# tayloreisman16/LTE-GNU-Radio-Code

Hardware: AMD Instinct MI355X
Metric: IQ Msamples/s through RX FFT+equalize, 2048-pt/144-CP; %HBM roofline; 1/2/4/8 GPU (higher is better)
Workload: dtype f32; 1 GPU; 2048-pt FFT / 144-CP / Kd=1200 / 16-QAM, 4369 frames x 240 symbols (1,048,560 symbols), AWGN loopback; frames_per_gpu=4369, symbols_per_gpu=1048560, outputs=equalised symbols + packed bits, parallelism=frame-shard x1, sync_search=screened

## Files before the change

lte-gnu-radio-code_amd/csrc/rx_demod.hpp:

```cpp
#pragma once
#include <algorithm>
#include <atomic>
#include <cstdlib>
#include <type_traits>

#include "ofdm_launch.hpp"

#ifndef OFDM_NS_T128
#define OFDM_NS_T128 2
#endif
#ifndef OFDM_MINW_T128
#define OFDM_MINW_T128 3
#endif
#ifndef OFDM_FLAGS_T128
#define OFDM_FLAGS_T128 0u
#endif
#ifndef OFDM_FLAGS_T256
#define OFDM_FLAGS_T256 0u
#endif
#ifndef OFDM_LANE_TW
#define OFDM_LANE_TW 1
#endif
#ifndef OFDM_SCATTER_HOIST
#define OFDM_SCATTER_HOIST 1
#endif
#ifndef OFDM_SCATTER_SKIP
#define OFDM_SCATTER_SKIP 1
#endif

namespace ofdm {

__device__ __forceinline__ unsigned qpsk_axis_bit(float x) {
    constexpr float t = 1.41421354f;
    return unsigned(x < 0.f) ^ unsigned(fabsf(x) > t);
}

__device__ __noinline__ unsigned qpsk_bits_on_axis(float zx, float zy) {
    constexpr double A = 0x1.6a09e667f3bcdp-1, B = 0x1.6a09e667f3bccp-1, Cc = 0x1.6a09e667f3bcep-1;
    const double cx[4] = {A, A, -B, -Cc};
    const double cy[4] = {B, -B, A, -B};
    constexpr double K = 0x1.6a09e667f3bccp+0;
    const double x = double(zx), y = double(zy);
    int kbest = 0;
    double dbest = 0.0;
#pragma unroll
    for (int k = 0; k < 4; ++k) {
        const double ax = fabs(x - cx[k]), ay = fabs(y - cy[k]);
        const double mx = fmax(ax, ay), mn = fmin(ay, ax);
        const double r = mn / mx;
        const double d = sqrt(fma(r, r, 1.0)) * mx;
        if (k == 0 || d < dbest) {
            dbest = d;
            kbest = k;
        }
    }
    const double ex = fabs(x - cx[kbest]), ey = fabs(y - cy[kbest]);
    const bool q1 = x >= 0.0 && y >= 0.0;
    const bool q2 = !q1 && x <= 0.0 && y >= 0.0;
    const bool q3 = !q1 && !q2 && x <= 0.0 && y <= 0.0;
    const bool q4 = !q1 && !q2 && !q3 && x >= 0.0 && y <= 0.0;
    const bool re_pos = q1 || q4, im_pos = q1 || q2;
    const double fr = K - ex, fi = K - ey;
    const unsigned b0 = re_pos ? (fr < ex) : (ex < fr);
    const unsigned b1 = im_pos ? (fi < ey) : (ey < fi);
    return (b0 << 1) | b1;
}

template <int MOD>
__device__ __forceinline__ unsigned hard_bits(cf z) {
    if constexpr (MOD == 2) {
        if (z.x == 0.f || z.y == 0.f) return qpsk_bits_on_axis(z.x, z.y);
        return (qpsk_axis_bit(z.x) << 1) | qpsk_axis_bit(z.y);
    } else if constexpr (MOD == 1) {
        return z.x > 0.f;
    } else if constexpr (MOD == 4) {
        constexpr float t = 0.63245553203367588f;
        return (unsigned(z.x < 0.f) << 3) | (unsigned(z.y < 0.f) << 2) | (unsigned(fabsf(z.x) > t) << 1) |
               unsigned(fabsf(z.y) > t);
    } else {
        constexpr float a = 0.61721339984836765f;
        constexpr float c = 0.30860669992418382f;
        return (unsigned(z.x < 0.f) << 5) | (unsigned(z.y < 0.f) << 4) | (unsigned(fabsf(z.x) > a) << 3) |
               (unsigned(fabsf(z.y) > a) << 2) | (unsigned(fabsf(fabsf(z.x) - a) > c) << 1) |
               unsigned(fabsf(fabsf(z.y) - a) > c);
    }
}
__device__ __forceinline__ unsigned hard_bits_rt(cf z, int mod) {
    return mod == 2 ? hard_bits<2>(z) : mod == 1 ? hard_bits<1>(z) : mod == 4 ? hard_bits<4>(z) : hard_bits<6>(z);
}

template <int MOD, bool ASMB = true>
__device__ __forceinline__ unsigned pack4(const cf (&z)[4]) {
    unsigned w = 0;
    if constexpr (!ASMB) {
        w = (((((hard_bits<MOD>(z[0]) << MOD) | hard_bits<MOD>(z[1])) << MOD) | hard_bits<MOD>(z[2])) << MOD) | hard_bits<MOD>(z[3]);
    } else if constexpr (MOD == 4) {
        constexpr float t = 0.63245553203367588f;
        unsigned long long m0, m1, m2, m3;
#define OFDM_Q16(RE, IM)                                   \
    "v_cmp_gt_f32_e64 %1, 0, " RE "\n\t"                   \
    "v_cmp_gt_f32_e64 %2, 0, " IM "\n\t"                   \
    "v_cmp_gt_f32_e64 %3, |" RE "|, %13\n\t"               \
    "v_cmp_gt_f32_e64 %4, |" IM "|, %13\n\t"               \
    "v_addc_co_u32_e64 %0, %1, %0, %0, %1\n\t"             \
    "v_addc_co_u32_e64 %0, %2, %0, %0, %2\n\t"             \
    "v_addc_co_u32_e64 %0, %3, %0, %0, %3\n\t"             \
    "v_addc_co_u32_e64 %0, %4, %0, %0, %4\n\t"
        asm(OFDM_Q16("%5", "%6") OFDM_Q16("%7", "%8") OFDM_Q16("%9", "%10") OFDM_Q16("%11", "%12")
            : "+v"(w), "=&s"(m0), "=&s"(m1), "=&s"(m2), "=&s"(m3)
            : "v"(z[0].x), "v"(z[0].y), "v"(z[1].x), "v"(z[1].y), "v"(z[2].x), "v"(z[2].y), "v"(z[3].x), "v"(z[3].y), "s"(t));
#undef OFDM_Q16
    } else if constexpr (MOD == 6) {
        constexpr float a = 0.61721339984836765f;
        constexpr float c = 0.30860669992418382f;
        unsigned long long m0, m1, m2, m3, m4, m5;
        float tr, ti;
#define OFDM_Q64(RE, IM)                                   \
    "v_sub_f32_e64 %7, |" RE "|, %17\n\t"                  \
    "v_sub_f32_e64 %8, |" IM "|, %17\n\t"                  \
    "v_cmp_gt_f32_e64 %1, 0, " RE "\n\t"                   \
    "v_cmp_gt_f32_e64 %2, 0, " IM "\n\t"                   \
    "v_cmp_gt_f32_e64 %3, |" RE "|, %17\n\t"               \
    "v_cmp_gt_f32_e64 %4, |" IM "|, %17\n\t"               \
    "v_cmp_gt_f32_e64 %5, |%7|, %18\n\t"                   \
    "v_cmp_gt_f32_e64 %6, |%8|, %18\n\t"                   \
    "v_addc_co_u32_e64 %0, %1, %0, %0, %1\n\t"             \
    "v_addc_co_u32_e64 %0, %2, %0, %0, %2\n\t"             \
    "v_addc_co_u32_e64 %0, %3, %0, %0, %3\n\t"             \
    "v_addc_co_u32_e64 %0, %4, %0, %0, %4\n\t"             \
    "v_addc_co_u32_e64 %0, %5, %0, %0, %5\n\t"             \
    "v_addc_co_u32_e64 %0, %6, %0, %0, %6\n\t"
        asm(OFDM_Q64("%9", "%10") OFDM_Q64("%11", "%12") OFDM_Q64("%13", "%14") OFDM_Q64("%15", "%16")
            : "+v"(w), "=&s"(m0), "=&s"(m1), "=&s"(m2), "=&s"(m3), "=&s"(m4), "=&s"(m5), "=&v"(tr), "=&v"(ti)
            : "v"(z[0].x), "v"(z[0].y), "v"(z[1].x), "v"(z[1].y), "v"(z[2].x), "v"(z[2].y), "v"(z[3].x), "v"(z[3].y), "s"(a), "s"(c));
#undef OFDM_Q64
    } else if constexpr (MOD == 2) {
        constexpr float t = 1.41421354f;
        if (!(fabsf(z[0].x * z[0].y * z[1].x * z[1].y) > 0.f) || !(fabsf(z[2].x * z[2].y * z[3].x * z[3].y) > 0.f)) {
            bool tie = false;
#pragma unroll
            for (int e = 0; e < 4; ++e) tie |= (z[e].x == 0.f) | (z[e].y == 0.f);
            if (tie)
                return (((((hard_bits<2>(z[0]) << 2) | hard_bits<2>(z[1])) << 2) | hard_bits<2>(z[2])) << 2) | hard_bits<2>(z[3]);
        }
        unsigned long long m0, m1, m2, m3, m4, m5, m6, m7;
#define OFDM_QPSK2(RE0, IM0, RE1, IM1)                     \
    "v_cmp_gt_f32_e64 %1, 0, " RE0 "\n\t"                  \
    "v_cmp_gt_f32_e64 %2, |" RE0 "|, %17\n\t"              \
    "v_cmp_gt_f32_e64 %3, 0, " IM0 "\n\t"                  \
    "v_cmp_gt_f32_e64 %4, |" IM0 "|, %17\n\t"              \
    "v_cmp_gt_f32_e64 %5, 0, " RE1 "\n\t"                  \
    "v_cmp_gt_f32_e64 %6, |" RE1 "|, %17\n\t"              \
    "v_cmp_gt_f32_e64 %7, 0, " IM1 "\n\t"                  \
    "v_cmp_gt_f32_e64 %8, |" IM1 "|, %17\n\t"              \
    "s_xor_b64 %1, %1, %2\n\t"                             \
    "s_xor_b64 %3, %3, %4\n\t"                             \
    "s_xor_b64 %5, %5, %6\n\t"                             \
    "s_xor_b64 %7, %7, %8\n\t"                             \
    "s_nop 1\n\t"                                          \
    "v_addc_co_u32_e64 %0, %1, %0, %0, %1\n\t"             \
    "v_addc_co_u32_e64 %0, %3, %0, %0, %3\n\t"             \
    "v_addc_co_u32_e64 %0, %5, %0, %0, %5\n\t"             \
    "v_addc_co_u32_e64 %0, %7, %0, %0, %7\n\t"
        asm(OFDM_QPSK2("%9", "%10", "%11", "%12") OFDM_QPSK2("%13", "%14", "%15", "%16")
            : "+v"(w), "=&s"(m0), "=&s"(m1), "=&s"(m2), "=&s"(m3), "=&s"(m4), "=&s"(m5), "=&s"(m6), "=&s"(m7)
            : "v"(z[0].x), "v"(z[0].y), "v"(z[1].x), "v"(z[1].y), "v"(z[2].x), "v"(z[2].y), "v"(z[3].x), "v"(z[3].y), "s"(t)
            : "scc");
#undef OFDM_QPSK2
    } else {
        w = (((((hard_bits<MOD>(z[0]) << MOD) | hard_bits<MOD>(z[1])) << MOD) | hard_bits<MOD>(z[2])) << MOD) | hard_bits<MOD>(z[3]);
    }
    return w;
}

template <int MOD, bool ASMB = true>
__device__ __forceinline__ unsigned pack2(const cf (&z)[2]) {
    unsigned w = 0;
    if constexpr (!ASMB || MOD == 1) {
        w = (hard_bits<MOD>(z[0]) << MOD) | hard_bits<MOD>(z[1]);
    } else if constexpr (MOD == 4) {
        constexpr float t = 0.63245553203367588f;
        unsigned long long m0, m1, m2, m3;
#define OFDM_Q16(RE, IM)                                   \
    "v_cmp_gt_f32_e64 %1, 0, " RE "\n\t"                   \
    "v_cmp_gt_f32_e64 %2, 0, " IM "\n\t"                   \
    "v_cmp_gt_f32_e64 %3, |" RE "|, %9\n\t"                \
    "v_cmp_gt_f32_e64 %4, |" IM "|, %9\n\t"                \
    "v_addc_co_u32_e64 %0, %1, %0, %0, %1\n\t"             \
    "v_addc_co_u32_e64 %0, %2, %0, %0, %2\n\t"             \
    "v_addc_co_u32_e64 %0, %3, %0, %0, %3\n\t"             \
    "v_addc_co_u32_e64 %0, %4, %0, %0, %4\n\t"
        asm(OFDM_Q16("%5", "%6") OFDM_Q16("%7", "%8")
            : "+v"(w), "=&s"(m0), "=&s"(m1), "=&s"(m2), "=&s"(m3)
            : "v"(z[0].x), "v"(z[0].y), "v"(z[1].x), "v"(z[1].y), "s"(t));
#undef OFDM_Q16
    } else if constexpr (MOD == 6) {
        constexpr float a = 0.61721339984836765f;
        constexpr float c = 0.30860669992418382f;
        unsigned long long m0, m1, m2, m3, m4, m5;
        float tr, ti;
#define OFDM_Q64(RE, IM)                                   \
    "v_sub_f32_e64 %7, |" RE "|, %13\n\t"                  \
    "v_sub_f32_e64 %8, |" IM "|, %13\n\t"                  \
    "v_cmp_gt_f32_e64 %1, 0, " RE "\n\t"                   \
    "v_cmp_gt_f32_e64 %2, 0, " IM "\n\t"                   \
    "v_cmp_gt_f32_e64 %3, |" RE "|, %13\n\t"               \
    "v_cmp_gt_f32_e64 %4, |" IM "|, %13\n\t"               \
    "v_cmp_gt_f32_e64 %5, |%7|, %14\n\t"                   \
    "v_cmp_gt_f32_e64 %6, |%8|, %14\n\t"                   \
    "v_addc_co_u32_e64 %0, %1, %0, %0, %1\n\t"             \
    "v_addc_co_u32_e64 %0, %2, %0, %0, %2\n\t"             \
    "v_addc_co_u32_e64 %0, %3, %0, %0, %3\n\t"             \
    "v_addc_co_u32_e64 %0, %4, %0, %0, %4\n\t"             \
    "v_addc_co_u32_e64 %0, %5, %0, %0, %5\n\t"             \
    "v_addc_co_u32_e64 %0, %6, %0, %0, %6\n\t"
        asm(OFDM_Q64("%9", "%10") OFDM_Q64("%11", "%12")
            : "+v"(w), "=&s"(m0), "=&s"(m1), "=&s"(m2), "=&s"(m3), "=&s"(m4), "=&s"(m5), "=&v"(tr), "=&v"(ti)
            : "v"(z[0].x), "v"(z[0].y), "v"(z[1].x), "v"(z[1].y), "s"(a), "s"(c));
#undef OFDM_Q64
    } else {
        constexpr float t = 1.41421354f;
        if (!(fabsf(z[0].x * z[0].y * z[1].x * z[1].y) > 0.f)) {
            const bool tie = (z[0].x == 0.f) | (z[0].y == 0.f) | (z[1].x == 0.f) | (z[1].y == 0.f);
            if (tie) return (hard_bits<2>(z[0]) << 2) | hard_bits<2>(z[1]);
        }
        unsigned long long m0, m1, m2, m3, m4, m5, m6, m7;
        asm("v_cmp_gt_f32_e64 %1, 0, %9\n\t"
            "v_cmp_gt_f32_e64 %2, |%9|, %13\n\t"
            "v_cmp_gt_f32_e64 %3, 0, %10\n\t"
            "v_cmp_gt_f32_e64 %4, |%10|, %13\n\t"
            "v_cmp_gt_f32_e64 %5, 0, %11\n\t"
            "v_cmp_gt_f32_e64 %6, |%11|, %13\n\t"
            "v_cmp_gt_f32_e64 %7, 0, %12\n\t"
            "v_cmp_gt_f32_e64 %8, |%12|, %13\n\t"
            "s_xor_b64 %1, %1, %2\n\t"
            "s_xor_b64 %3, %3, %4\n\t"
            "s_xor_b64 %5, %5, %6\n\t"
            "s_xor_b64 %7, %7, %8\n\t"
            "s_nop 1\n\t"
            "v_addc_co_u32_e64 %0, %1, %0, %0, %1\n\t"
            "v_addc_co_u32_e64 %0, %3, %0, %0, %3\n\t"
            "v_addc_co_u32_e64 %0, %5, %0, %0, %5\n\t"
            "v_addc_co_u32_e64 %0, %7, %0, %0, %7\n\t"
            : "+v"(w), "=&s"(m0), "=&s"(m1), "=&s"(m2), "=&s"(m3), "=&s"(m4), "=&s"(m5), "=&s"(m6), "=&s"(m7)
            : "v"(z[0].x), "v"(z[0].y), "v"(z[1].x), "v"(z[1].y), "s"(t)
            : "scc");
    }
    return w;
}

template <int MOD>
__device__ __forceinline__ void store_bits_pair_unpacked(uint8_t* row, unsigned sym0, const cf (&z)[2]) {
    uint8_t* o = row + sym0 * unsigned(MOD);
#pragma unroll
    for (int e = 0; e < 2; ++e) {
        const unsigned hb = hard_bits<MOD>(z[e]);
#pragma unroll
        for (int b = 0; b < MOD; ++b) o[e * MOD + b] = uint8_t((hb >> (MOD - 1 - b)) & 1u);
    }
}

template <int MOD>
__device__ __forceinline__ void store_packed4(uint8_t* row, unsigned sym0, unsigned w) {
    uint8_t* o = row + (sym0 >> 2) * unsigned(MOD / 2);
    if constexpr (MOD == 2) {
        o[0] = uint8_t(w);
    } else if constexpr (MOD == 4) {
        *reinterpret_cast<uint16_t*>(o) = uint16_t(((w & 0xffu) << 8) | (w >> 8));
    } else {
        o[0] = uint8_t(w >> 16);
        o[1] = uint8_t(w >> 8);
        o[2] = uint8_t(w);
    }
}

template <int MOD, int BMODE, bool ASMB = true>
__device__ __forceinline__ void store_bits(uint8_t* bits, int64_t sym0, const cf (&z)[4], int cnt) {
    if constexpr (BMODE == 1) {
        store_packed4<MOD>(bits + (sym0 >> 2) * (MOD / 2), 0u, pack4<MOD, ASMB>(z));
    } else if constexpr (BMODE == 2) {
        uint8_t* o = bits + sym0 * MOD;
#pragma unroll
        for (int e = 0; e < 4; ++e) {
            if (e < cnt) {
                const unsigned hb = hard_bits<MOD>(z[e]);
#pragma unroll
                for (int b = 0; b < MOD; ++b) o[e * MOD + b] = uint8_t((hb >> (MOD - 1 - b)) & 1u);
            }
        }
    }
}

template <int N>
struct DemodGeom {
    static constexpr int T = Plan<N>::T;
    static constexpr int NS = (T >= 256) ? 1 : (T >= 128) ? OFDM_NS_T128 : (T >= 64 ? 2 : 64 / T);
    static constexpr int WG = T * NS;
    static constexpr int W1_OFF = WgLds<N>::STRIDE * NS;
    static constexpr int Q_OFF = W1_OFF + WgLds<N>::W1_ELEMS;
    static constexpr int G_OFF = Q_OFF + 2;
    static size_t lds_bytes(int Kd, bool glds) { return (size_t(G_OFF) + (glds ? ((Kd + 3) & ~3) : 0)) * sizeof(cf); }
    static constexpr int KD_LTE = (N >= 1024) ? N * 75 / 128 : 0;
};

enum DemodFlags : unsigned {
    DF_ROT = 1u << 0,
    DF_HG = 1u << 1,
    DF_UNITS = 1u << 15,
    DF_GAINS_GLOBAL = 1u << 2,
    DF_TEMPORAL_LD = 1u << 3,
    DF_TEMPORAL_ST = 1u << 11,
    DF_GENERIC_BITS = 1u << 4,
    DF_STAMP = 1u << 5,
    DF_NO_PIPE = 1u << 6,
    DF_L2_INPUT = 1u << 7,
    DF_LANE_TWIDDLES = 1u << 8,
    DF_PSUM_READBACK = 1u << 9,
    DF_GAINS_VGPR = 1u << 14,
    DF_FOUR_PER_LANE = 1u << 10,
};

template <int N, int MOD, int BMODE, int MINW, unsigned FLAGS = 0, int KD = 0>
__global__ void __launch_bounds__(DemodGeom<N>::WG, MINW) rx_demod_kernel(RxDev rx, DemodArgs a) {
    static_assert(KD >= 0 && KD <= N && KD % 4 == 0, "compile-time bin-list length");
    constexpr bool ROT = (FLAGS & DF_ROT) != 0, HG = (FLAGS & DF_HG) != 0, UNITS = (FLAGS & DF_UNITS) != 0,
                   GREG = (FLAGS & DF_GAINS_VGPR) != 0 && Plan<N>::T >= 64 && (FLAGS & DF_FOUR_PER_LANE) == 0 && !(MOD == 1 && BMODE == 1),
                   GLDS = (FLAGS & DF_GAINS_GLOBAL) == 0 && !GREG,
                   NTL = (FLAGS & DF_TEMPORAL_LD) == 0 && Plan<N>::T >= 64, NT = (FLAGS & DF_TEMPORAL_ST) == 0 && Plan<N>::T >= 64, ASMB = (FLAGS & DF_GENERIC_BITS) == 0, STAMP = (FLAGS & DF_STAMP) != 0,
                   PIPE = (FLAGS & DF_NO_PIPE) == 0, L2IN = (FLAGS & DF_L2_INPUT) != 0,
                   CT = (FLAGS & DF_LANE_TWIDDLES) == 0 && !OFDM_LANE_TW && Plan<N>::R0 == 16, PSE = (FLAGS & DF_PSUM_READBACK) == 0,
                   DENSE = Plan<N>::T >= 64 && (FLAGS & DF_FOUR_PER_LANE) == 0 && !(MOD == 1 && BMODE == 1);
    using PL = Plan<N>;
    using DG = DemodGeom<N>;
    constexpr int T = PL::T, P = PL::P, Q = P / 4, NS = DG::NS;
    extern __shared__ __attribute__((aligned(16))) char smem_raw[];
    const int tid = threadIdx.x;
    const int slot = (T >= 64) ? __builtin_amdgcn_readfirstlane(tid / T) : tid / T;
    const int t = tid % T;
    constexpr bool WL = T <= 64;
    cf* smem = reinterpret_cast<cf*>(smem_raw);
    cf* lds = smem + slot * WgLds<N>::STRIDE;
    float* red = reinterpret_cast<float*>(lds + WgLds<N>::ELEMS);
    cf* w1w = smem + DG::W1_OFF;
    if constexpr (PL::THREE) {
        for (int e = tid; e < WgLds<N>::W1_ELEMS; e += DG::WG) w1w[e] = w1_entry<N>(rx.tw, e);
    }
    const cf* w1tab = w1w;

    std::conditional_t<CT, CompactTwiddles<N>, LaneTwiddles<N>> tw;
    load_twiddles(tw, rx.tw, t);

    unsigned acc[8] = {0, 0, 0, 0, 0, 0, 0, 0};
    unsigned long long tprev = 0;
    auto stamp = [&](int i) {
        if constexpr (STAMP) {
            unsigned long long tn;
            asm volatile("s_memtime %0\n\ts_waitcnt lgkmcnt(0)" : "=s"(tn)::"memory");
            acc[i] += unsigned(tn - tprev);
            tprev = tn;
        }
    };
    if constexpr (STAMP) asm volatile("s_memtime %0\n\ts_waitcnt lgkmcnt(0)" : "=s"(tprev)::"memory");
    const int64_t n_chunks = int64_t(a.n_frames) * a.chunks_per_frame;
    int* const qslot = reinterpret_cast<int*>(smem + DG::Q_OFF);
    int64_t chunk = blockIdx.x;
    if (a.work) {
        if (tid == 0) *qslot = int(atomicAdd(a.work, 1u));
        __syncthreads();
        chunk = *qslot;
    }
    for (; chunk < n_chunks;) {
    const int frame = int(chunk / a.chunks_per_frame);
    const int cidx = int(chunk % a.chunks_per_frame);
    const int trips = (a.n_dsym + NS - 1) / NS;
    const int ds0 = int(int64_t(cidx) * trips / a.chunks_per_frame) * NS;
    const int ds1 = min(int(int64_t(cidx + 1) * trips / a.chunks_per_frame) * NS, a.n_dsym);
    constexpr bool active = true;

    const int Kd = KD > 0 ? KD : rx.Kd, L = rx.L, S = rx.S, D = rx.D;
    const int tsr0 = a.tsr[frame * 4 + 0];
    const bool frame_on = (HG || UNITS) ? (a.tsr[frame * 4 + 3] != 0) : true;
    const int src_frame = UNITS ? frame / a.units_per_frame : frame;
    const cf* frame_iq = a.iq + int64_t(L2IN ? (blockIdx.x & 7) : src_frame) * a.frame_stride;
    const cf* rotp = (UNITS && ROT) ? a.rot + int64_t(max(a.rot_idx[src_frame], 0)) * N : a.rot;

    const cf* gain = a.gain + int64_t(frame) * Kd;
    cf* glds = smem + DG::G_OFF;
    const cf* gsrc = GLDS ? glds : gain;
    if constexpr (GLDS) {
        for (int i = 2 * tid; i < Kd; i += 2 * DG::WG) *reinterpret_cast<float4*>(glds + i) = *reinterpret_cast<const float4*>(gain + i);
    }
    float4 greg[GREG ? Q : 1][2];
    if constexpr (GREG) {
#pragma unroll
        for (int q = 0; q < Q; ++q)
#pragma unroll
            for (int hx = 0; hx < 2; ++hx) {
                const int idx = 4 * T * q + 256 * (t >> 6) + 128 * hx + 2 * (t & 63);
                greg[q][hx] = idx < Kd ? *reinterpret_cast<const float4*>(gain + idx) : float4{0.f, 0.f, 0.f, 0.f};
            }
    }

    const float sqrt_kd = sqrtf(float(Kd));
    const int n_iter = (ds1 - ds0 + NS - 1) / NS;
    struct Sym {
        bool valid, compute;
        int64_t start, orow;
    };
    auto sym_of = [&](int it) {
        Sym sy;
        const int itr = it;
        const int ds = ds0 + itr * NS + slot;
        sy.valid = active && it < n_iter && ds < ds1;
        const int p = ds / D, n_ = ds - p * D;
        const int64_t pat_ptr = int64_t(tsr0) + int64_t(S) * L * (int64_t(p) * (S + D) + 1);
        sy.compute = sy.valid && (HG ? frame_on : (pat_ptr + N - 1 <= a.frame_len)) && (!UNITS || frame_on);
        sy.start = pat_ptr + int64_t(L) * n_;
        sy.orow = int64_t(frame) * a.rows_per_frame + (p * a.row_stride_pat + n_);
        return sy;
    };
    cf v[P];
    auto load_sym = [&](const Sym& sy) {
        if (sy.compute && sy.start >= 0 && sy.start + N <= a.frame_len) {
            const cf* src = frame_iq + sy.start + t;
#pragma unroll
            for (int n0 = 0; n0 < P; ++n0) v[n0] = NTL ? __builtin_nontemporal_load(src + T * n0) : src[T * n0];
            if constexpr (ROT) {
#pragma unroll
                for (int n0 = 0; n0 < P; ++n0) v[n0] = cmul(v[n0], rotp[t + T * n0]);
            }
        } else {
            const int64_t before = -sy.start, left = a.frame_len - sy.start;
            const int lo = int(before < 0 ? 0 : (before < N ? before : N)), hi = int(left < 0 ? 0 : (left < N ? left : N));
            const bool any = sy.compute && hi > lo;
            int tq = t;
            asm volatile("" : "+v"(tq));
#pragma unroll
            for (int n0 = 0; n0 < P; ++n0) {
                const int e = tq + T * n0;
                const cf x = any ? frame_iq[sy.start + min(max(e, lo), hi - 1)] : cf{0.f, 0.f};
                v[n0] = (any && e >= lo && e < hi) ? x : cf{0.f, 0.f};
                if constexpr (ROT) v[n0] = cmul(v[n0], rotp[tq + T * n0]);
            }
        }
    };

    Sym cur = sym_of(0);
    if constexpr (PIPE) load_sym(cur);
    if constexpr (WL) wg_barrier();
    for (int it = 0; it < n_iter; ++it) {
        if constexpr (!PIPE) {
            cur = sym_of(it);
            load_sym(cur);
        }
        const bool sym_valid = cur.valid, compute = cur.compute;
        const int64_t orow = cur.orow;
        stamp(0);
        if constexpr (STAMP) asm volatile("s_waitcnt vmcnt(0)" ::: "memory");
        stamp(1);
        if constexpr (STAMP) {
            fft_pass0_store<N>(v, lds, tw, t);
            wg_barrier();
            stamp(2);
            if constexpr (PL::THREE) {
                fft_pass1_load<N>(v, lds, t);
                wg_barrier();
                fft_pass1_store<N>(v, lds, w1tab, t);
                wg_barrier();
            }
            stamp(3);
            fft_last_load<N>(v, lds, t);
            fft_last_dft<N>(v);
        } else {
            wg_fft<N, decltype(tw), WL>(v, lds, tw, w1tab, t);
        }
        slot_sync<WL>();

        int Kd_ = Kd;
#if !OFDM_SCATTER_HOIST
        asm volatile("" : "+s"(Kd_));
#endif
        const int hk = Kd_ >> 1;
        const int off_neg = hk - N, off_pos = hk - 1;
        float pse = 0.f;
#pragma unroll
        for (int j = 0; j < PL::C; ++j) {
#pragma unroll
            for (int kl = 0; kl < PL::RL; ++kl) {
#if OFDM_SCATTER_SKIP
                if constexpr (T >= 64) {
                    const int base = T * j + PL::NC * kl;
                    if (base > hk && base + T - 1 < N - hk) continue;
                }
#endif
                const int k = (t + T * j) + PL::NC * kl;
#if OFDM_SCATTER_SKIP
                if constexpr (T >= 64) {
                    const int base = T * j + PL::NC * kl;
                    const bool all_pos = base >= 1 && base + T - 1 <= hk, all_neg = base >= N - hk && hk < N / 2;
                    if (all_pos || all_neg) {
                        lds[k + (all_neg ? off_neg : off_pos)] = v[out_slot<N>(j, kl)];
                        if constexpr (PSE) pse += cnorm2(v[out_slot<N>(j, kl)]);
                        continue;
                    }
                }
#endif
                int i = k + ((k >= N - hk) ? off_neg : off_pos);
                if (j == 0 && kl == 0) i = (k == 0) ? N : i;
                lds[i] = v[out_slot<N>(j, kl)];
                if constexpr (PSE) pse += (unsigned(i) < unsigned(Kd_)) ? cnorm2(v[out_slot<N>(j, kl)]) : 0.f;
            }
        }
        if (Kd_ == N) {
#pragma unroll
            for (int j = 0; j < PL::C; ++j) {
#pragma unroll
                for (int kl = 0; kl < PL::RL; ++kl)
                    if ((t + T * j) + PL::NC * kl == N / 2) {
                        lds[N - 1] = v[out_slot<N>(j, kl)];
                        if constexpr (PSE) pse += cnorm2(v[out_slot<N>(j, kl)]);
                    }
            }
        }
        if constexpr (PSE) {
            pse = lanes_sum<T>(pse);
            if constexpr (T > 64) {
                if ((t & 63) == 0) red[t >> 6] = pse;
            }
        }
        slot_sync<WL>();

        stamp(4);
        if constexpr (PIPE) {
            cur = sym_of(it + 1);
            load_sym(cur);
        }
        float psum = 0.f;
        if constexpr (PSE) {
            if constexpr (T > 64) {
#pragma unroll
                for (int w = 0; w < T / 64; ++w) psum += red[w];
            } else {
                psum = pse;
            }
        } else {
#pragma unroll
            for (int q = 0; q < Q; ++q) {
                const int idx = 4 * (t + T * q);
                const float4 a01 = *reinterpret_cast<const float4*>(lds + idx);
                const float4 a23 = *reinterpret_cast<const float4*>(lds + idx + 2);
                const float p4[4] = {a01.x * a01.x + a01.y * a01.y, a01.z * a01.z + a01.w * a01.w,
                                     a23.x * a23.x + a23.y * a23.y, a23.z * a23.z + a23.w * a23.w};
                if (4 * T * (q + 1) <= Kd_) {
#pragma unroll
                    for (int e = 0; e < 4; ++e) psum += p4[e];
                } else {
#pragma unroll
                    for (int e = 0; e < 4; ++e) psum += (idx + e < Kd_) ? p4[e] : 0.f;
                }
            }
            psum = lanes_sum<T>(psum);
            if constexpr (T > 64) {
                if ((t & 63) == 0) red[t >> 6] = psum;
                wg_barrier();
                psum = 0.f;
#pragma unroll
                for (int w = 0; w < T / 64; ++w) psum += red[w];
            }
        }
        const float scale = sqrt_kd * __builtin_amdgcn_rsqf(psum);
        stamp(5);

        if (!compute) {
            if (sym_valid && a.zero_skipped) {
                const cf zz[4] = {cf{0.f, 0.f}, cf{0.f, 0.f}, cf{0.f, 0.f}, cf{0.f, 0.f}};
                int tq = t;
                asm volatile("" : "+v"(tq));
#pragma unroll
                for (int q = 0; q < Q; ++q) {
                    const int idx = 4 * (tq + T * q);
                    if (idx < Kd_) {
                        const bool four = idx + 2 < Kd_;
                        if (a.eq) {
                            float4* o = reinterpret_cast<float4*>(a.eq + orow * Kd_ + idx);
                            o[0] = float4{0.f, 0.f, 0.f, 0.f};
                            if (four) o[1] = float4{0.f, 0.f, 0.f, 0.f};
                        }
                        if constexpr (BMODE != 0) store_bits<MOD, BMODE>(a.bits, orow * Kd_ + idx, zz, four ? 4 : 2);
                    }
                }
            }
        } else if constexpr (DENSE) {
            const int wv = __builtin_amdgcn_readfirstlane(t >> 6), ln = t & 63;
            const int lane_e = ((t >> 6) << 8) + 2 * ln;
            const int64_t row0 = orow * Kd_;
            cf* const eq_row = a.eq ? a.eq + row0 : nullptr;
            uint8_t* const bits_row = (BMODE == 0) ? nullptr : (BMODE == 1) ? a.bits + ((row0 * MOD) >> 3) : a.bits + row0 * MOD;
            const cf* const l_lane = lds + lane_e;
            const cf* const g_lane = gsrc + lane_e;
            const unsigned eq_off = unsigned(lane_e) * unsigned(sizeof(cf));
            const int lnm = (KD > 0) ? opaque_lane(ln) : ln;
#pragma unroll
            for (int q = 0; q < Q; ++q) {
                const int b0 = 4 * T * q + 256 * wv;
                if (b0 < Kd_) {
                    unsigned wp[2] = {0u, 0u};
#pragma unroll
                    for (int hx = 0; hx < 2; ++hx) {
                        const int base = b0 + 128 * hx;
                        const int cofs = 4 * T * q + 128 * hx;
                        auto pair = [&]() {
                            float4 g;
                            if constexpr (GREG)
                                g = greg[q][hx];
                            else
                                g = *reinterpret_cast<const float4*>(g_lane + cofs);
                            const float4 av = *reinterpret_cast<const float4*>(l_lane + cofs);
                            cf z[2] = {cf{av.x, av.y} * scale, cf{av.z, av.w} * scale};
                            cmul2(z[0], cf{g.x, g.y}, z[1], cf{g.z, g.w});
                            if (eq_row) {
                                typedef float f4 __attribute__((ext_vector_type(4)));
                                const f4 ov = f4{z[0].x, z[0].y, z[1].x, z[1].y};
                                cf* const blk = eq_row + cofs;
#ifdef OFDM_EXPERIMENTS
                                constexpr unsigned SPOL = (FLAGS >> 12) & 3u;
                                if constexpr (SPOL == 1) {
                                    asm volatile("global_store_dwordx4 %0, %1, %2 sc1" ::"v"(eq_off), "v"(ov), "s"(blk) : "memory");
                                } else if constexpr (SPOL == 2) {
                                    asm volatile("global_store_dwordx4 %0, %1, %2 sc0 sc1" ::"v"(eq_off), "v"(ov), "s"(blk) : "memory");
                                } else if constexpr (SPOL == 3) {
                                    asm volatile("global_store_dwordx4 %0, %1, %2 sc0 sc1 nt" ::"v"(eq_off), "v"(ov), "s"(blk) : "memory");
                                } else
#endif
                                if constexpr (NT) {
                                    asm volatile("global_store_dwordx4 %0, %1, %2 nt" ::"v"(eq_off), "v"(ov), "s"(blk) : "memory");
                                } else {
                                    asm volatile("global_store_dwordx4 %0, %1, %2" ::"v"(eq_off), "v"(ov), "s"(blk) : "memory");
                                }
                            }
                            if constexpr (BMODE == 1) wp[hx] = pack2<MOD, ASMB>(z);
                            if constexpr (BMODE == 2) store_bits_pair_unpacked<MOD>(bits_row + cofs * MOD, unsigned(lane_e), z);
                        };
                        if (base + 128 <= Kd_) {
                            pair();
                        } else if (base < Kd_) {
                            if (base + 2 * lnm < Kd_) pair();
                        }
                    }
                    if constexpr (BMODE == 1) {
                        const bool odd = (ln & 1) != 0;
                        const unsigned recv = unsigned(__builtin_amdgcn_mov_dpp(int(odd ? wp[0] : wp[1]), 0xB1, 0xF, 0xF, false));
                        const unsigned w4 = odd ? ((recv << (2 * MOD)) | wp[1]) : ((wp[0] << (2 * MOD)) | recv);
                        const int ge = lane_e + (odd ? 126 : 0);
                        uint8_t* const brow = bits_row + (4 * T * q / 4) * (MOD / 2);
                        if (b0 + 256 <= Kd_) {
                            store_packed4<MOD>(brow, unsigned(ge), w4);
                        } else if (4 * T * q + ((KD > 0) ? opaque_lane(ge) : ge) < Kd_) {
                            store_packed4<MOD>(brow, unsigned(ge), w4);
                        }
                    }
                }
            }
        } else {
#pragma unroll
            for (int q = 0; q < Q; ++q) {
                const int idx = 4 * (t + T * q);
                if (idx < Kd_) {
                    const bool four = idx + 2 < Kd_;
                    const float4 g01 = *reinterpret_cast<const float4*>(gsrc + idx);
                    const float4 g23 = (GLDS || four) ? *reinterpret_cast<const float4*>(gsrc + idx + 2) : float4{0.f, 0.f, 0.f, 0.f};
                    const float4 a01 = *reinterpret_cast<const float4*>(lds + idx);
                    const float4 a23 = *reinterpret_cast<const float4*>(lds + idx + 2);
                    cf z[4] = {cf{a01.x, a01.y} * scale, cf{a01.z, a01.w} * scale, cf{a23.x, a23.y} * scale,
                               cf{a23.z, a23.w} * scale};
                    cmul3(z[0], cf{g01.x, g01.y}, z[1], cf{g01.z, g01.w}, z[2], cf{g23.x, g23.y});
                    z[3] = cmul(z[3], cf{g23.z, g23.w});
                    if (a.eq) {
                        float4* o = reinterpret_cast<float4*>(a.eq + orow * Kd_ + idx);
                        const float4 o0 = float4{z[0].x, z[0].y, z[1].x, z[1].y}, o1 = float4{z[2].x, z[2].y, z[3].x, z[3].y};
                        if constexpr (NT) {
                            typedef float f4 __attribute__((ext_vector_type(4)));
                            f4* on = reinterpret_cast<f4*>(o);
                            __builtin_nontemporal_store(f4{o0.x, o0.y, o0.z, o0.w}, on);
                            if (four) __builtin_nontemporal_store(f4{o1.x, o1.y, o1.z, o1.w}, on + 1);
                        } else {
                            o[0] = o0;
                            if (four) o[1] = o1;
                        }
                    }
                    if constexpr (BMODE != 0) store_bits<MOD, BMODE, ASMB>(a.bits, orow * Kd_ + idx, z, four ? 4 : 2);
                }
            }
        }
        stamp(6);
        slot_sync<WL>();
        stamp(7);
    }
    if (!a.work) break;
    __syncthreads();
    if (tid == 0) *qslot = int(atomicAdd(a.work, 1u));
    __syncthreads();
    chunk = *qslot;
    }
    if (a.work) {
        if (tid == 0 && atomicAdd(a.work + 1, 1u) == gridDim.x - 1) {
            atomicExch(a.work, 0u);
            atomicExch(a.work + 1, 0u);
        }
    }
    if constexpr (STAMP) {
        if ((tid & 63) == 0 && a.stamps) {
            unsigned* o = a.stamps + (int64_t(blockIdx.x) * (DG::WG / 64) + (tid >> 6)) * 8;
#pragma unroll
            for (int i = 0; i < 8; ++i) o[i] = acc[i];
        }
    }
}

template <int N, int KD>
hipError_t launch_rx_demod_batch(const RxDev& rx, DemodArgs a, unsigned grid, size_t lds, int bmode, hipStream_t s) {
    using DG = DemodGeom<N>;
    constexpr int MW = (Plan<N>::T == 128) ? OFDM_MINW_T128 : 3;
    constexpr unsigned FL = (Plan<N>::T == 128) ? OFDM_FLAGS_T128 : (Plan<N>::T == 256) ? OFDM_FLAGS_T256 : 0u;
#define OFDM_LD(M, B)                                                                                                        \
    do {                                                                                                                     \
        static std::atomic<int> announced{65536};                \
        if (int(lds) > announced.load(std::memory_order_relaxed)) {                                                          \
            hipError_t e = hipFuncSetAttribute(reinterpret_cast<const void*>(&rx_demod_kernel<N, M, B, MW, FL, KD>),         \
                                               hipFuncAttributeMaxDynamicSharedMemorySize, int(lds));                       \
            if (e != hipSuccess) return e;                                                                                   \
            announced.store(int(lds), std::memory_order_relaxed);                                                            \
        }                                                                                                                    \
        hipLaunchKernelGGL((rx_demod_kernel<N, M, B, MW, FL, KD>), dim3(grid), dim3(DG::WG), lds, s, rx, a);                 \
    } while (0)
    if (N < 1024) a.work = nullptr;
    if (a.work) {
        static int per_cu = 0, n_cu = 0;
        if (per_cu == 0) {
            int nb = 0, dev = 0;
            hipDeviceProp_t prop;
            if (hipOccupancyMaxActiveBlocksPerMultiprocessor(&nb, rx_demod_kernel<N, 4, 1, MW, FL, KD>, DG::WG, lds) != hipSuccess || nb < 1) nb = 2;
            n_cu = (hipGetDevice(&dev) == hipSuccess && hipGetDeviceProperties(&prop, dev) == hipSuccess && prop.multiProcessorCount > 0)
                       ? prop.multiProcessorCount : 256;
            per_cu = nb;
        }
        const int64_t resident = int64_t(per_cu) * n_cu;
        if (int64_t(grid) > 2 * resident)
            grid = unsigned(resident);
        else
            a.work = nullptr;
    }
#define OFDM_LD_MOD(B)                  \
    switch (a.mod) {                    \
        case 1: OFDM_LD(1, B); break;   \
        case 2: OFDM_LD(2, B); break;   \
        case 4: OFDM_LD(4, B); break;   \
        default: OFDM_LD(6, B); break;  \
    }
    if (bmode == 0) {
        OFDM_LD(2, 0);
    } else if (bmode == 1) {
        OFDM_LD_MOD(1)
    } else {
        OFDM_LD_MOD(2)
    }
#undef OFDM_LD_MOD
#undef OFDM_LD
    return hipGetLastError();
}

#define OFDM_EXTERN_DEMOD_KD(n) \
    extern template hipError_t launch_rx_demod_batch<n, DemodGeom<n>::KD_LTE>(const RxDev&, DemodArgs, unsigned, size_t, int, hipStream_t);
OFDM_EXTERN_DEMOD_KD(1024)
OFDM_EXTERN_DEMOD_KD(2048)
OFDM_EXTERN_DEMOD_KD(4096)
#undef OFDM_EXTERN_DEMOD_KD

template <int N>
hipError_t launch_rx_demod_n(const RxDev& rx, const DemodArgs& a_in, hipStream_t s) {
    using DG = DemodGeom<N>;
    DemodArgs a = a_in;
    if (a.n_frames <= 0 || a.n_dsym <= 0) return hipSuccess;
    if (a.chunks_per_frame <= 0) {
        const int trips = (a.n_dsym + DG::NS - 1) / DG::NS;
        const int64_t total_trips = int64_t(a.n_frames) * trips;
        const int per_chunk = N == 2048 ? 20 : N >= 4096 ? 14 : N == 1024 ? 12 : std::max(12, 131072 / (rx.L * 8));
        int want = int(std::max<int64_t>(1, (int64_t(trips) * DG::NS + per_chunk - 1) / per_chunk));
        if (total_trips / std::max(want, 1) < 4096) want = int(std::max<int64_t>(1, std::min<int64_t>(trips, 4096 / std::max(a.n_frames, 1))));
#ifdef OFDM_TUNE_ENV
        if (const char* e = getenv("OFDM_DEMOD_CPF")) want = atoi(e);
#endif
        want = std::max(1, std::min(want, trips));
        int best = want;
        if (trips % want != 0) {
            best = 0;
            for (int d = 0; d <= want / 2 && !best; ++d) {
                if (want + d <= trips && trips % (want + d) == 0) best = want + d;
                else if (want - d >= 1 && trips % (want - d) == 0 && 3 * (want - d) >= 2 * want) best = want - d;
            }
            if (!best) best = (want & 1) ? want : std::min(want + 1, trips);
        }
        a.chunks_per_frame = best;
        a.spc = ((trips + best - 1) / best) * DG::NS;
    }
    unsigned grid = unsigned(int64_t(a.n_frames) * a.chunks_per_frame);
    size_t lds = DG::lds_bytes(rx.Kd, !((Plan<N>::T == 128 && (OFDM_FLAGS_T128 & (DF_GAINS_GLOBAL | DF_GAINS_VGPR))) ||
                                        (Plan<N>::T == 256 && (OFDM_FLAGS_T256 & (DF_GAINS_GLOBAL | DF_GAINS_VGPR)))));
#ifdef OFDM_EXPERIMENTS
    if (a.variant >= 100) lds += size_t(a.variant - 100) * 1024;
#endif
    const int bmode = a.bits ? a.bits_mode : 0;
    if (a.host_guard) {
        if (bmode != 0 || a.rot) return hipErrorInvalidValue;
        hipLaunchKernelGGL((rx_demod_kernel<N, 2, 0, 3, DF_HG>), dim3(grid), dim3(DG::WG), lds, s, rx, a);
        return hipGetLastError();
    }
    if (a.units_per_frame > 0) {
        if (a.mod != 2 || a.host_guard || a.work || (a.rot && !a.rot_idx)) return hipErrorInvalidValue;
#define OFDM_FO_UNITS(B, FL)                                                                                                 \
    do {                                                                                                                     \
        if (lds > 65536) {                                                                                                   \
            hipError_t e = hipFuncSetAttribute(reinterpret_cast<const void*>(&rx_demod_kernel<N, 2, B, 2, DF_UNITS | FL>),   \
                                               hipFuncAttributeMaxDynamicSharedMemorySize, int(lds));                       \
            if (e != hipSuccess) return e;                                                                                   \
        }                                                                                                                    \
        hipLaunchKernelGGL((rx_demod_kernel<N, 2, B, 2, DF_UNITS | FL>), dim3(grid), dim3(DG::WG), lds, s, rx, a);           \
    } while (0)
        if (a.rot) {
            if (bmode == 0) OFDM_FO_UNITS(0, DF_ROT);
            else if (bmode == 1) OFDM_FO_UNITS(1, DF_ROT);
            else OFDM_FO_UNITS(2, DF_ROT);
        } else {
            if (bmode == 0) OFDM_FO_UNITS(0, 0u);
            else if (bmode == 1) OFDM_FO_UNITS(1, 0u);
            else OFDM_FO_UNITS(2, 0u);
        }
#undef OFDM_FO_UNITS
        return hipGetLastError();
    }
    if (a.rot) {
        if (bmode != 0) return hipErrorInvalidValue;
        hipLaunchKernelGGL((rx_demod_kernel<N, 2, 0, 3, DF_ROT>), dim3(grid), dim3(DG::WG), lds, s, rx, a);
        return hipGetLastError();
    }
#ifdef OFDM_EXPERIMENTS
    if constexpr (N == 2048) {
        if ((a.variant == 13 || a.variant == 1) && bmode == 1 && a.mod != 4) {
            constexpr unsigned PLAIN = DF_TEMPORAL_LD | DF_TEMPORAL_ST;
            if (a.mod == 6 && a.variant == 13)
                hipLaunchKernelGGL((rx_demod_kernel<N, 6, 1, 3, DF_FOUR_PER_LANE | PLAIN>), dim3(grid), dim3(DG::WG), lds, s, rx, a);
            else if (a.mod == 6)
                hipLaunchKernelGGL((rx_demod_kernel<N, 6, 1, 3, PLAIN>), dim3(grid), dim3(DG::WG), lds, s, rx, a);
            else if (a.variant == 13)
                hipLaunchKernelGGL((rx_demod_kernel<N, 2, 1, 3, DF_FOUR_PER_LANE | PLAIN>), dim3(grid), dim3(DG::WG), lds, s, rx, a);
            else
                hipLaunchKernelGGL((rx_demod_kernel<N, 2, 1, 3, PLAIN>), dim3(grid), dim3(DG::WG), lds, s, rx, a);
            return hipGetLastError();
        }
        if (a.variant != 0 && a.variant < 100 && bmode == 1 && a.mod == 4) {
#define OFDM_LV(V, MW, FL, LDSB)                                                                                            \
    if (a.variant == V) {                                                                                                   \
        hipLaunchKernelGGL((rx_demod_kernel<N, 4, 1, MW, FL>), dim3(grid), dim3(DG::WG), LDSB, s, rx, a);                   \
        return hipGetLastError();                                                                                           \
    }
            OFDM_LV(1, 3, DF_TEMPORAL_LD | DF_TEMPORAL_ST, lds)
            OFDM_LV(14, 3, DF_TEMPORAL_ST, lds)
            OFDM_LV(21, 3, 1u << 12, lds)
            OFDM_LV(22, 3, 2u << 12, lds)
            OFDM_LV(23, 3, 3u << 12, lds)
            OFDM_LV(15, 3, DF_TEMPORAL_LD, lds)
            OFDM_LV(2, 3, DF_GAINS_GLOBAL, DG::lds_bytes(rx.Kd, false))
            OFDM_LV(3, 3, DF_GENERIC_BITS, lds)
            OFDM_LV(5, 3, DF_NO_PIPE, lds)
            OFDM_LV(6, 3, DF_L2_INPUT, lds)
            OFDM_LV(8, 4, 0u, lds)
            OFDM_LV(9, 3, DF_STAMP, lds)
            OFDM_LV(10, 3, DF_LANE_TWIDDLES | DF_PSUM_READBACK, lds)
            OFDM_LV(11, 3, DF_PSUM_READBACK, lds)
            OFDM_LV(12, 3, DF_LANE_TWIDDLES, lds)
            OFDM_LV(13, 3, DF_FOUR_PER_LANE | DF_TEMPORAL_LD | DF_TEMPORAL_ST, lds)
#undef OFDM_LV
        }
    }
#endif
    if constexpr (DemodGeom<N>::KD_LTE > 0) {
        if (rx.Kd == DemodGeom<N>::KD_LTE) return launch_rx_demod_batch<N, DemodGeom<N>::KD_LTE>(rx, a, grid, lds, bmode, s);
    }
    return launch_rx_demod_batch<N, 0>(rx, a, grid, lds, bmode, s);
}

#define OFDM_DECLARE_DEMOD(n) hipError_t launch_rx_demod_##n(const RxDev& rx, const DemodArgs& a, hipStream_t s);
OFDM_DECLARE_DEMOD(64)
OFDM_DECLARE_DEMOD(128)
OFDM_DECLARE_DEMOD(256)
OFDM_DECLARE_DEMOD(512)
OFDM_DECLARE_DEMOD(1024)
OFDM_DECLARE_DEMOD(2048)
OFDM_DECLARE_DEMOD(4096)
#undef OFDM_DECLARE_DEMOD

}
```

Measured before the change: 587,300 Msamples/s.

## Issue symbol loads via inline asm with counted vmcnt waits for overlap

On the dense path, the next symbol's 16 input loads are issued as inline-asm global_load_dwordx2 with immediate offsets off a shared scalar base. Before the FFT, the code waits with an s_waitcnt vmcnt that depends on how many equalised-output stores were issued since those loads, rather than draining everything. The aim is to let outstanding stores stay in flight while the prefetched symbol arrives, and to cut address arithmetic. The risk is that the hand-counted vmcnt bookkeeping is fragile. If the compiler emits other vector-memory operations, the count could be wrong and the wait could fall short.

Result: slower. 578,900 Msamples/s (-1.4%).

```diff
diff --git a/lte-gnu-radio-code_amd/csrc/rx_demod.hpp b/lte-gnu-radio-code_amd/csrc/rx_demod.hpp
--- a/lte-gnu-radio-code_amd/csrc/rx_demod.hpp
+++ b/lte-gnu-radio-code_amd/csrc/rx_demod.hpp
@@ -3,6 +3,7 @@
 #include <atomic>
 #include <cstdlib>
 #include <type_traits>
+#include <utility>
 
 #include "ofdm_launch.hpp"
 
@@ -291,6 +292,54 @@
     }
 }
 
+
+template <int IMM, bool NTL>
+__device__ __forceinline__ void stream_load_cf(cf& d, unsigned voff, const char* sbase) {
+    static_assert(IMM >= -4096 && IMM <= 4095, "global_load immediate offset");
+    if constexpr (NTL)
+        asm volatile("global_load_dwordx2 %0, %1, %2 offset:%3 nt" : "=v"(d) : "v"(voff), "s"(sbase), "n"(IMM));
+    else
+        asm volatile("global_load_dwordx2 %0, %1, %2 offset:%3" : "=v"(d) : "v"(voff), "s"(sbase), "n"(IMM));
+}
+template <int T, bool NTL, int... I>
+__device__ __forceinline__ void stream_load_sym(cf (&v)[16], unsigned voff, const cf* src, std::integer_sequence<int, I...>) {
+    const char* const b = reinterpret_cast<const char*>(src);
+    (stream_load_cf<T * 8 * I - ((T * 8 * I) / 8192 * 8192 + 4096), NTL>(v[I], voff, b + ((T * 8 * I) / 8192 * 8192 + 4096)), ...);
+}
+#define OFDM_V16(v)                                                                                                          \
+    "+v"(v[0]), "+v"(v[1]), "+v"(v[2]), "+v"(v[3]), "+v"(v[4]), "+v"(v[5]), "+v"(v[6]), "+v"(v[7]), "+v"(v[8]), "+v"(v[9]), \
+        "+v"(v[10]), "+v"(v[11]), "+v"(v[12]), "+v"(v[13]), "+v"(v[14]), "+v"(v[15])
+__device__ __forceinline__ void stream_wait_counted(cf (&v)[16], unsigned newer) {
+    asm volatile(
+        "s_cmp_lt_u32 %[n], 2\n\t"
+        "s_cbranch_scc1 .Lsw0_%=\n\t"
+        "s_cmp_lt_u32 %[n], 4\n\t"
+        "s_cbranch_scc1 .Lsw2_%=\n\t"
+        "s_cmp_lt_u32 %[n], 6\n\t"
+        "s_cbranch_scc1 .Lsw4_%=\n\t"
+        "s_cmp_lt_u32 %[n], 8\n\t"
+        "s_cbranch_scc1 .Lsw6_%=\n\t"
+        "s_waitcnt vmcnt(8)\n\t"
+        "s_branch .Lswe_%=\n"
+        ".Lsw6_%=:\n\t"
+        "s_waitcnt vmcnt(6)\n\t"
+        "s_branch .Lswe_%=\n"
+        ".Lsw4_%=:\n\t"
+        "s_waitcnt vmcnt(4)\n\t"
+        "s_branch .Lswe_%=\n"
+        ".Lsw2_%=:\n\t"
+        "s_waitcnt vmcnt(2)\n\t"
+        "s_branch .Lswe_%=\n"
+        ".Lsw0_%=:\n\t"
+        "s_waitcnt vmcnt(0)\n"
+        ".Lswe_%=:"
+        : OFDM_V16(v)
+        : [n] "s"(__builtin_amdgcn_readfirstlane(newer))
+        : "scc");
+}
+__device__ __forceinline__ void stream_wait_all(cf (&v)[16]) { asm volatile("s_waitcnt vmcnt(0)" : OFDM_V16(v)); }
+#undef OFDM_V16
+
 template <int N>
 struct DemodGeom {
     static constexpr int T = Plan<N>::T;
@@ -330,6 +379,7 @@
                    PIPE = (FLAGS & DF_NO_PIPE) == 0, L2IN = (FLAGS & DF_L2_INPUT) != 0,
                    CT = (FLAGS & DF_LANE_TWIDDLES) == 0 && !OFDM_LANE_TW && Plan<N>::R0 == 16, PSE = (FLAGS & DF_PSUM_READBACK) == 0,
                    DENSE = Plan<N>::T >= 64 && (FLAGS & DF_FOUR_PER_LANE) == 0 && !(MOD == 1 && BMODE == 1);
+    constexpr bool CW = DENSE && !ROT && !HG && !UNITS;
     using PL = Plan<N>;
     using DG = DemodGeom<N>;
     constexpr int T = PL::T, P = PL::P, Q = P / 4, NS = DG::NS;
@@ -420,11 +470,17 @@
         return sy;
     };
     cf v[P];
+    unsigned newer = 0;
     auto load_sym = [&](const Sym& sy) {
+        newer = 0;
         if (sy.compute && sy.start >= 0 && sy.start + N <= a.frame_len) {
-            const cf* src = frame_iq + sy.start + t;
-#pragma unroll
-            for (int n0 = 0; n0 < P; ++n0) v[n0] = NTL ? __builtin_nontemporal_load(src + T * n0) : src[T * n0];
+            if constexpr (CW) {
+                stream_load_sym<T, NTL>(v, unsigned(t) * unsigned(sizeof(cf)), frame_iq + sy.start, std::make_integer_sequence<int, P>{});
+            } else {
+                const cf* src = frame_iq + sy.start + t;
+#pragma unroll
+                for (int n0 = 0; n0 < P; ++n0) v[n0] = NTL ? __builtin_nontemporal_load(src + T * n0) : src[T * n0];
+            }
             if constexpr (ROT) {
 #pragma unroll
                 for (int n0 = 0; n0 < P; ++n0) v[n0] = cmul(v[n0], rotp[t + T * n0]);
@@ -441,6 +497,9 @@
                 const cf x = any ? frame_iq[sy.start + min(max(e, lo), hi - 1)] : cf{0.f, 0.f};
                 v[n0] = (any && e >= lo && e < hi) ? x : cf{0.f, 0.f};
                 if constexpr (ROT) v[n0] = cmul(v[n0], rotp[tq + T * n0]);
+            }
+            if constexpr (CW) {
+                if (any) stream_wait_all(v);
             }
         }
     };
@@ -456,7 +515,10 @@
         const bool sym_valid = cur.valid, compute = cur.compute;
         const int64_t orow = cur.orow;
         stamp(0);
-        if constexpr (STAMP) asm volatile("s_waitcnt vmcnt(0)" ::: "memory");
+        if constexpr (CW)
+            stream_wait_counted(v, newer);
+        else if constexpr (STAMP)
+            asm volatile("s_waitcnt vmcnt(0)" ::: "memory");
         stamp(1);
         if constexpr (STAMP) {
             fft_pass0_store<N>(v, lds, tw, t);
@@ -646,6 +708,7 @@
                         } else if (base < Kd_) {
                             if (base + 2 * lnm < Kd_) pair();
                         }
+                        if constexpr (CW) newer += unsigned(eq_row != nullptr && base < Kd_);
                     }
                     if constexpr (BMODE == 1) {
                         const bool odd = (ln & 1) != 0;
```
